# JuliaGenAI/ColBERT.jl

Hardware: AMD Instinct MI355X
Metric: queries/sec, top-1000 on 1M-passage corpus (higher is better)
Workload: dtype f32

## Files before the change

### colbert.jl_amd/csrc/approx_kernels.hpp

```cpp
#pragma once
#include <hip/hip_fp16.h>

#include <algorithm>

#include "common.hpp"
#include "search_kernels.hpp"

namespace clb {

typedef __bf16 bf16x8 __attribute__((ext_vector_type(8)));
typedef uint32_t u32x4 __attribute__((ext_vector_type(4)));
typedef uint32_t u32x4_a4 __attribute__((ext_vector_type(4), aligned(4)));
typedef float f32x4_a4 __attribute__((ext_vector_type(4), aligned(4)));

constexpr float kEpsSafety = 1.25f;

inline bool approx_supported(int dim, int nbits) { return dim == kDim && nbits == 2; }
inline size_t approx_cells_bytes(int64_t B, int64_t K, int64_t ) { return (size_t)B * K * 16 * 4 + 2048; }

__device__ __forceinline__ uint32_t f32_to_bf16_rne(float f) {
    const uint32_t u = __float_as_uint(f);
    return (u + 0x7fffu + ((u >> 16) & 1u)) >> 16;
}
__device__ __forceinline__ uint32_t pack_bf16(float lo, float hi) {
// ... 1213 lines not shown
    float rb_max;
    float dw_rn;
    float inv_qerr;
    float dc_max;
};

struct QueryBound { float eps_t, eps_sum; bool unsafe; };
__device__ __forceinline__ QueryBound query_bound(const float* __restrict__ Q, int b, int T, const ApproxConsts& ac,
                                                  float* s_qn, float* s_dq, const float4* __restrict__ tscale = nullptr,
                                                  float* s_aux = nullptr ,
                                                  bool cell8 = false) {
    const int tid = threadIdx.x;
    if (tid == 0) { *s_qn = 0.f; *s_dq = 0.f; }
    if (tscale && tid < 4) s_aux[tid] = 0.f;
    __syncthreads();
    {
        const int t = tid >> 5, part = tid & 31;
        float a = 0.f, dd = 0.f, d8 = 0.f;
        if (t < T) {
            const float4 v = *reinterpret_cast<const float4*>(Q + ((size_t)b * T + t) * kDim + 4 * part);
            a = fmaf(v.x, v.x, fmaf(v.y, v.y, fmaf(v.z, v.z, v.w * v.w)));
            const float dx = v.x - round_f16(v.x), dy = v.y - round_f16(v.y);
            const float dz = v.z - round_f16(v.z), dw = v.w - round_f16(v.w);
            dd = fmaf(dx, dx, fmaf(dy, dy, fmaf(dz, dz, dw * dw)));
            if (tscale && cell8) {
                const float4 ts = tscale[(size_t)b * 32 + t];
                const float sx = v.x * ts.y, sy = v.y * ts.y, sz = v.z * ts.y, sw = v.w * ts.y;
                const float ex = sx - round_f16(sx), ey = sy - round_f16(sy), ez = sz - round_f16(sz), ew = sw - round_f16(sw);
                d8 = fmaf(ex, ex, fmaf(ey, ey, fmaf(ez, ez, ew * ew)));
            }
        }
#pragma unroll
// ... 25 lines not shown
            const float dq8 = s_aux[0], step_max = s_aux[1];
            e_tab = e_f16 + 0.5005f * step_max + 8.f * u * amax;
            e_qr = 1.001f * ((dq8 + 2.f * u * qn) * ac.rb_max + qn * ac.dw_rn) +
                   2.f * 130.f * u * (amax + 255.f * step_max + qn * ac.rn_max) + 1280.f * u * step_max;
            bad8 = s_aux[2] != 0.f;
        }
    }
    const float eps_t = (ac.inv_max + ac.inv_qerr) * (e_tab + e_qr) + 1.01f * ac.inv_qerr * qn * (ac.cn_max + ac.rn_max) + 332.f * u * qn;
    QueryBound r;
    r.eps_t = eps_t;
    r.unsafe = !(qn * ac.cn_max < 3.0e4f) || !(qn < 6.0e4f)  || !(eps_t < 1.0e30f) || bad8;
    r.eps_sum = kEpsSafety * ((float)T * eps_t + 2.f * (float)T * (float)T * u * qn);
    return r;
}

static __global__ __launch_bounds__(1024) void select_margin_kernel(const float* __restrict__ scores,
                                                                   const int* __restrict__ ncand,
                                                                   const float* __restrict__ Q, int T, int k,
                                                                   size_t cand_cap, ApproxConsts ac,
                                                                   int* __restrict__ list, int* __restrict__ nlist,
                                                                   float* __restrict__ thresh,
                                                                   float* __restrict__ eps_pair,
                                                                   const float* __restrict__ tau_in = nullptr,
                                                                   int coarse_tau = 0,
                                                                   const float4* __restrict__ tscale = nullptr,
                                                                   int cell8 = 0) {
    __shared__ __attribute__((aligned(16))) int hist[256];
    __shared__ float s_aux[4];
    __shared__ int sh_scan[16];
    __shared__ int sh_big[2][8][16];
    __shared__ uint32_t s_prefix, s_kmin, s_kmax;
    __shared__ int s_remaining, s_run;
    __shared__ float s_qn, s_dq;
    const int b = blockIdx.x, tid = threadIdx.x;
    const int n = ncand[b];
    const float* sc = scores + (size_t)b * cand_cap;
    int* lst = list + (size_t)b * cand_cap;
    if (tid == 0) { s_prefix = 0u; s_remaining = n < k ? n : k; s_run = 0; }
    const int chunk = (n + 1023) >> 10;
    const int i0 = tid * chunk;
    const bool cached = chunk <= kSelCache;
    uint32_t ckey[kSelCache];
    if (cached) {
#pragma unroll
        for (int c = 0; c < kSelCache; ++c) ckey[c] = (c < chunk && i0 + c < n) ? f32_order_key(sc[i0 + c]) : 0u;
    }
    const QueryBound qb = query_bound(Q, b, T, ac, &s_qn, &s_dq, tscale, s_aux, cell8 != 0);
    float thr = kNegInf, tau_f = kNegInf, eps = 0.f;
    const bool unsafe = qb.unsafe;
    if (tid == 0) eps_pair[b] = unsafe ? __builtin_inff() : kEpsSafety * qb.eps_t;
#define CLB_SEL_FOR_EACH(...)                                                                   \
    if (cached) {                                                                               \
        _Pragma("unroll") for (int c = 0; c < kSelCache; ++c) {                                 \
            if (c >= chunk) break;                                                              \
            const int i = i0 + c;                                                               \
            const bool valid = i < n;                                                           \
            const uint32_t key = ckey[c];                                                       \
            __VA_ARGS__                                                                         \
        }                                                                                       \
    } else {    \
        _Pragma("unroll 4") for (int c = 0; c < chunk; ++c) {                                   \
            const int i = c * 1024 + tid;                                                       \
            const bool valid = i < n;                                                           \
            const uint32_t key = valid ? f32_order_key(sc[i]) : 0u;                             \
            __VA_ARGS__                                                                         \
// ... 148 lines not shown
                    st.shift = ns;
                }
            }
            __syncthreads();
        }
    }
    return st;
}

static __global__ __launch_bounds__(1024) void wide_minmax_kernel(const float* __restrict__ scores,
                                                                 const int* __restrict__ ncand,
                                                                 const float* __restrict__ Q, int T, size_t cand_cap,
                                                                 ApproxConsts ac, WideSel* __restrict__ wsel,
                                                                 float* __restrict__ eps_pair,
                                                                 const float4* __restrict__ tscale = nullptr,
                                                                 int cell8 = 0) {
    __shared__ uint32_t s_kmin, s_kmax;
    __shared__ float s_qn, s_dq, s_aux[4];
    const int b = blockIdx.y, g = blockIdx.x, tid = threadIdx.x;
    const int n = ncand[b];
    const float* sc = scores + (size_t)b * cand_cap;
    WideSel& w = wsel[b];
    if (tid == 0) { s_kmin = 0xffffffffu; s_kmax = 0u; }
    __syncthreads();
    if (g == 0) {
        const QueryBound qb = query_bound(Q, b, T, ac, &s_qn, &s_dq, tscale, s_aux, cell8 != 0);
        if (tid == 0) {
            eps_pair[b] = qb.unsafe ? __builtin_inff() : kEpsSafety * qb.eps_t;
            w.unsafe = qb.unsafe ? 1 : 0;
            w.eps_sum = qb.eps_sum;
        }
    }
    int lo, hi;
    wide_segment(n, g, lo, hi);
    uint32_t kmin = 0xffffffffu, kmax = 0u;
#pragma unroll 4
    for (int i = lo + tid; i < hi; i += 1024) {
        const uint32_t key = f32_order_key(sc[i]);
        kmin = key < kmin ? key : kmin;
        kmax = key > kmax ? key : kmax;
// ... 271 lines not shown
```

### colbert.jl_amd/csrc/search.hip

```cpp
#include <algorithm>
#include <atomic>
#include <cstdlib>
#include <cstring>
#include <numeric>

#include "approx_kernels.hpp"
#include "generic_kernels.hpp"
#include "search_kernels.hpp"
#include "sort.hpp"

using namespace clb;

namespace {

enum KernelId {
    KID_CENTROID_SCORES = 0,
    KID_TOPN,
    KID_MARK,
    KID_COMPACT,
    KID_SCORE_EXACT,
    KID_SCORE_APPROX,
    KID_SELECT,
    KID_ROWS,
    KID_TOPK,
// ... 34 lines not shown
    DevBuf bits;
};

struct Workspace {
    int64_t Bcap = 0, Tcap = 0, npcap = 0, kcap = 0;
    int64_t Ttuned = 0;
    size_t cand_cap = 0;
    int W = 0, nblk_bitmap = 0, topn_blocks = 0;
    bool x1_table = false;
    bool have_range = false;
    bool cell8 = false;
    size_t filt_cap = 0;
    size_t ivf_cap = 0;
    struct { bool valid = false; const float* dQ = nullptr; int64_t T = 0, B = 0, nprobe = 0, k = 0; void* stream = nullptr; } pending;
    DevBuf Qdev, cells, cells_q, partial, sel, bitmap, blocksum, ncand, cand, cand_hdr, scores, list, nlist, thresh,
        outp, outs, flags, stats, redo, rowmask, eps_pair, tokmax, tau_glob, wsel, bounds, tscale, rangep, cells8;
    DevBuf g_cells, g_keys, g_keys2, g_vals, g_vals2, g_scratch, g_sort_tmp;
};

constexpr int kWorkspaceSlots = 4;

struct clb_searcher {
    int device = 0;
    uint64_t serial = 0;
    int64_t dim = 0, K = 0, n_docs = 0, n_emb = 0, pid_offset = 0;
    int nbits = 0;
    int mode = 0;
    int wide_select = -1;
    bool approx_ok = false;
    bool bounds_synced = false;
    bool ivf_sorted = false;
// ... 68 lines not shown
            s->prof.chain_stream = st;
        } else {
            s->prof.failed = true;
            s->prof.chain = nullptr;
        }
    }
};

inline int token_tiles(int64_t T) { return T <= 32 ? 1 : T <= 64 ? 2 : 4; }
inline int64_t padded_nprobe(int64_t nprobe) { return nprobe <= 2 ? 2 : nprobe <= 8 ? 8 : nprobe <= 32 ? 32 : nprobe; }

inline bool cell8_rows(const clb_searcher* s) { return s->cell8 == 1 && s->approx_ok; }

void allow_large_topk_lds() {
    allow_dynamic_lds(reinterpret_cast<const void*>(topk_kernel), (int)(sizeof(unsigned long long) * kMaxTopK));
}

constexpr int64_t kSubBatch = 64;

int next_pow2(int x) {
    int p = 1;
    while (p < x) p <<= 1;
    return p;
}

int ensure_workspace_sized(clb_searcher* s, Workspace& w, int64_t B, int64_t T, int64_t nprobe, int64_t k, size_t filt_count) {
    const int64_t t_tuned = T <= 128 ? T : 0;
    if (B <= w.Bcap && T <= w.Tcap && t_tuned <= w.Ttuned && nprobe <= w.npcap && k <= w.kcap && filt_count <= w.filt_cap)
        return CLB_OK;
    CLB_HIP(hipDeviceSynchronize());
// ... 37 lines not shown
    CLB_TRY(w.scores.ensure(sizeof(float) * B * w.cand_cap));
    CLB_TRY(w.list.ensure(sizeof(int) * B * w.cand_cap));
    CLB_TRY(w.nlist.ensure(sizeof(int) * B));
    CLB_TRY(w.thresh.ensure(sizeof(float) * B * 2));
    CLB_TRY(w.outp.ensure(sizeof(int64_t) * B * k));
    CLB_TRY(w.outs.ensure(sizeof(float) * B * k));
    CLB_TRY(w.flags.ensure(sizeof(int) * B));
    if (!w.stats.p) {
        CLB_TRY(w.stats.ensure(sizeof(unsigned long long) * 8));
        CLB_HIP(hipMemset(w.stats.p, 0, sizeof(unsigned long long) * 8));
    }
    if (s->approx_ok && Ttuned > 0) {
        CLB_TRY(w.cells_q.ensure(approx_cells_bytes(B, s->K, Tpad)));
        CLB_TRY(w.rowmask.ensure(sizeof(unsigned long long) * 4 * B * w.cand_cap));
        CLB_TRY(w.eps_pair.ensure(sizeof(float) * B));
        CLB_TRY(w.tokmax.ensure(sizeof(uint16_t) * 32 * B * w.cand_cap));
    }
    w.Bcap = B; w.Tcap = T; w.Ttuned = Ttuned; w.npcap = nprobe; w.kcap = k;
    w.filt_cap = std::max(w.filt_cap, filt_count);
    CLB_HIP(hipStreamSynchronize(s->stream));
    return CLB_OK;
}

int ensure_workspace(clb_searcher* s, Workspace& w, int64_t B, int64_t T, int64_t nprobe, int64_t k, size_t filt_count = 0) {
    const int rc = ensure_workspace_sized(s, w, B, T, nprobe, k, filt_count);
    if (rc) {
        w.Bcap = 0;
        if (rc == CLB_ENOMEM && filt_count > w.filt_cap)
            return fail(CLB_EUNSUPPORTED, "no room for the candidate buffers of a filter of %zu passages (CLB_FILTER_ALL, %lld "
                                          "queries per pass): %s", filt_count, (long long)B, std::string(last_error()).c_str());
// ... 21 lines not shown
int select_by_sort(clb_searcher* s, Workspace& w, hipStream_t st, const float* cells, size_t stride_t, size_t stride_c,
                   int T, int nprobe, int NP, int* sel_b);

int select_top_nprobe(clb_searcher* s, Workspace& w, hipStream_t st, int B, int T, int Tpad, int nprobe) {
    const int NPs = (int)padded_nprobe(nprobe);
    if (NPs == 2) launch_topn<2>(s, w, st, B, Tpad);
    else if (NPs == 8) launch_topn<8>(s, w, st, B, Tpad);
    else if (NPs == 32) launch_topn<32>(s, w, st, B, Tpad);
    else
        for (int b = 0; b < B; ++b)
            CLB_TRY(select_by_sort(s, w, st, w.cells.as<float>() + (size_t)b * s->K * Tpad, 1, (size_t)Tpad, T, nprobe, NPs,
                                   w.sel.as<int>() + (size_t)b * Tpad * NPs));
    return CLB_OK;
}

int mark_and_compact(clb_searcher* s, Workspace& w, hipStream_t st, const Batch& q, int b0, int B, int Tpad, int NPs, bool timed);

int run_retrieve(clb_searcher* s, Workspace& w, hipStream_t st, const Batch& q) {
    const float* dQ = q.dQ;
    const int B = q.B, T = q.T, nprobe = q.nprobe;
    const int TT = token_tiles(T), Tpad = TT * 32;
    const int n_tiles = (int)((s->K + 31) / 32);
    const bool want_half = s->mode == 1 && s->approx_ok && T <= 32;
    w.x1_table = false;
    w.have_range = false;
    w.cell8 = false;
    if (nprobe <= 2 && T <= 32) {
        const bool mq = B >= 6;
        const int groups = (B + kMqQueries - 1) / kMqQueries;
        int gx = mq ? std::max(1, std::min(n_tiles, std::min(256, std::max(512 / groups, 16))))
                          : std::max(1, std::min(n_tiles / 2 + 1, std::min(256, std::max(1024 / std::max(1, B), 16))));
// ... 62 lines not shown
            Timed t(s, KID_CENTROID_SCORES, st);
            const int gx = std::max(1, std::min(n_tiles / 2 + 1, 2048 / std::max(1, B * TT)));
            hipLaunchKernelGGL(centroid_scores_kernel, dim3(gx, B * TT), dim3(128),
                               2 * 32 * kCentTileStride * sizeof(float), st, s->centroids.as<float>(), dQ,
                               w.cells.as<float>(), (int)s->K, T, TT, n_tiles);
        }
        {
            Timed t(s, KID_TOPN, st);
            CLB_TRY(select_top_nprobe(s, w, st, B, T, Tpad, nprobe));
        }
        s->prof.chain = nullptr;
        if (want_half)
            hipLaunchKernelGGL(cells_to_half_kernel, dim3(std::max(1, 1024 / B), B), dim3(256), 0, st,
                               w.cells.as<float>(), w.cells_q.as<uint32_t>(), (int)s->K);
    }
    return mark_and_compact(s, w, st, q, 0, B, Tpad, (int)padded_nprobe(nprobe), true);
}

FilterArgs filter_args(const Batch& q, int b0, int n) {
    FilterArgs fa{};
    for (int i = 0; i < n && i < kFilterQueries; ++i) fa.bits[i] = q.filt[b0 + i] ? q.filt[b0 + i]->bits.as<uint32_t>() : nullptr;
    fa.all = q.filt_all;
    return fa;
}

template <bool FILT>
int mark_and_compact_impl(clb_searcher* s, Workspace& w, hipStream_t st, const Batch& q, int b0, int B, int Tpad, int NPs,
                          bool timed) {
    static_assert(kScanBlock * kWordsPerThread == 1024, "mark_count_kernel writes 1024-word count blocks");
    static_assert(kSubBatch <= kFilterQueries, "the filter handles of a sub-batch travel in one kernel argument block");
    FilterOperand<FILT> fa{};
    if constexpr (FILT) fa = filter_args(q, b0, B);
    const int T = q.T, nprobe = q.nprobe;
    uint32_t* bitmap = w.bitmap.as<uint32_t>() + (size_t)b0 * w.W;
    int* blocksum = w.blocksum.as<int>() + (size_t)b0 * w.nblk_bitmap;
    uint32_t* cand = w.cand.as<uint32_t>() + (size_t)b0 * w.cand_cap;
    uint2* cand_hdr = w.cand_hdr.as<uint2>() + (size_t)b0 * w.cand_cap;
    int* ncand = w.ncand.as<int>() + b0;
    const int nslices = (w.nblk_bitmap + kMarkSliceBlocks - 1) / kMarkSliceBlocks;
    const int nslices_big = (w.nblk_bitmap + kMarkSliceBlocksBig - 1) / kMarkSliceBlocksBig;
    const bool sliced = (nslices <= 16 || s->ivf_sorted) && B >= 8;
    {
        Timed t(s, timed ? KID_MARK : -1, st);
// ... 5 lines not shown
            const int nb = T * nprobe * (nslices_big + 1);
            hipLaunchKernelGGL(slice_bounds_kernel, dim3((nb + 255) / 256, B), dim3(256), 0, st, w.sel.as<int>(),
                               s->ivf_off.as<uint32_t>(), s->ivf_pid.as<uint32_t>(), T, Tpad, NPs, nprobe, nslices_big,
                               (uint32_t)(kMarkSliceBlocksBig * 1024 * 32), w.bounds.as<uint32_t>());
            hipLaunchKernelGGL((mark_count_kernel<true, kMarkSliceBlocksBig, FILT>), dim3(nslices_big, B), dim3(1024), 0, st,
                               w.sel.as<int>(), s->ivf_off.as<uint32_t>(), s->ivf_pid.as<uint32_t>(), bitmap, blocksum, T, Tpad,
                               NPs, nprobe, w.W, w.nblk_bitmap, (const uint32_t*)w.bounds.as<uint32_t>(), fa);
        } else
            hipLaunchKernelGGL(mark_candidates_kernel<FILT>, dim3(T * nprobe, B), dim3(256), 0, st, w.sel.as<int>(),
                               s->ivf_off.as<uint32_t>(), s->ivf_pid.as<uint32_t>(), bitmap, T, Tpad, NPs, nprobe, w.W, fa);
    }
    {
        Timed t(s, timed ? KID_COMPACT : -1, st);
        if (!sliced)
            hipLaunchKernelGGL(bitmap_count_kernel<FILT>, dim3(w.nblk_bitmap, B), dim3(kScanBlock), 0, st, bitmap, blocksum, w.W, fa);
        if (FILT && (!sliced || q.filt_all))
            hipLaunchKernelGGL(bitmap_emit_kernel<FILT>, dim3(w.nblk_bitmap, B), dim3(kScanBlock), 0, st, bitmap, blocksum, cand,
                               s->doc_off.as<uint32_t>(), cand_hdr, w.W, w.cand_cap, ncand, fa);
        else
            hipLaunchKernelGGL(bitmap_emit_kernel<false>, dim3(w.nblk_bitmap, B), dim3(kScanBlock), 0, st, bitmap, blocksum, cand,
                               s->doc_off.as<uint32_t>(), cand_hdr, w.W, w.cand_cap, ncand);
    }
    CLB_HIP(hipGetLastError());
    return CLB_OK;
}

int mark_and_compact(clb_searcher* s, Workspace& w, hipStream_t st, const Batch& q, int b0, int B, int Tpad, int NPs, bool timed) {
    bool filt = false;
    for (int b = b0; q.filt && b < b0 + B; ++b) filt |= q.filt[b] != nullptr;
    return filt ? mark_and_compact_impl<true>(s, w, st, q, b0, B, Tpad, NPs, timed)
                : mark_and_compact_impl<false>(s, w, st, q, b0, B, Tpad, NPs, timed);
}

int check_search_args(clb_searcher* s, int64_t T, int64_t B, int64_t nprobe, int64_t k) {
    if (!s) return fail(CLB_EARGUMENT, "null searcher");
    if (T < 1) return fail(CLB_EARGUMENT, "query length must be >= 1");
    if (B < 1) return fail(CLB_EARGUMENT, "batch size must be >= 1");
    if (nprobe < 1 || nprobe > s->K) return fail(CLB_EBOUNDS, "nprobe=%lld outside 1..K=%lld (partialsortperm)", (long long)nprobe, (long long)s->K);
    if (k < 1) return fail(CLB_EBOUNDS, "k must be >= 1");
    if (T * nprobe > (int64_t)0x7fffffff / 4 || T * s->K > (int64_t)0x7fffffff) return fail(CLB_EUNSUPPORTED, "T * K too large");
    return CLB_OK;
}

int select_by_sort(clb_searcher* s, Workspace& w, hipStream_t st, const float* cells, size_t stride_t, size_t stride_c,
                   int T, int nprobe, int NP, int* sel_b) {
    const size_t n = (size_t)T * s->K;
// ... 18 lines not shown
    const int* lst = list ? list + (size_t)b * w.cand_cap : nullptr;
    const int* n_ptr = list ? nlist + b : w.ncand.as<int>() + b;
    CLB_TRY(w.g_keys.ensure(sizeof(uint64_t) * std::max(cap, 1)));
    CLB_TRY(w.g_keys2.ensure(sizeof(uint64_t) * std::max(cap, 1)));
    hipLaunchKernelGGL(generic_topk_keys_kernel, dim3((cap + 255) / 256), dim3(256), 0, st, sc, lst, n_ptr, cap,
                       w.g_keys.as<unsigned long long>());
    CLB_TRY(sort_keys_u64(w.g_keys.as<uint64_t>(), w.g_keys2.as<uint64_t>(), (size_t)cap, st, &w.g_sort_tmp));
    hipLaunchKernelGGL(generic_topk_emit_kernel, dim3((std::max(k, 1) + 255) / 256), dim3(256), 0, st,
                       w.g_keys2.as<unsigned long long>(), sc, w.cand.as<uint32_t>() + (size_t)b * w.cand_cap, lst, n_ptr,
                       w.ncand.as<int>() + b, k, s->pid_offset, q.d_out_pids + (size_t)b * k, q.d_out_scores + (size_t)b * k,
                       w.flags.as<int>() + b, q.d_n_cand ? q.d_n_cand + b : nullptr);
    CLB_HIP(hipGetLastError());
    return CLB_OK;
}

int launch_topk(clb_searcher* s, Workspace& w, hipStream_t st, const Batch& q, int b0, int n, const int* list, const int* nlist,
                int ranked) {
    if (q.k > kMaxTopK) {
        for (int b = b0; b < b0 + n; ++b) CLB_TRY(topk_by_sort(s, w, st, q, b, list, nlist));
        return CLB_OK;
    }
    const int kpow2 = next_pow2(q.k);
    allow_large_topk_lds();
    hipLaunchKernelGGL(topk_kernel, dim3(n), dim3(1024), sizeof(unsigned long long) * kpow2, st,
                       w.scores.as<float>() + (size_t)b0 * w.cand_cap, w.cand.as<uint32_t>() + (size_t)b0 * w.cand_cap,
                       w.ncand.as<int>() + b0, list ? list + (size_t)b0 * w.cand_cap : nullptr, list ? nlist + b0 : nullptr, q.k, kpow2,
                       w.cand_cap, s->pid_offset, q.d_out_pids + (size_t)b0 * q.k, q.d_out_scores + (size_t)b0 * q.k,
                       w.flags.as<int>() + b0, q.d_n_cand ? q.d_n_cand + b0 : nullptr, ranked);
    CLB_HIP(hipGetLastError());
    return CLB_OK;
}

int run_retrieve_general(clb_searcher* s, Workspace& w, hipStream_t st, const Batch& q, int b) {
    const int T = q.T, nprobe = q.nprobe;
    CLB_TRY(w.g_cells.ensure(sizeof(float) * (size_t)T * s->K));
    hipLaunchKernelGGL(generic_cells_kernel, dim3((unsigned)((s->K + 127) / 128), T), dim3(128), sizeof(float) * s->dim, st,
                       s->centroids.as<float>(), q.dQ + (size_t)b * T * s->dim, (int)s->dim, (int)s->K, w.g_cells.as<float>());
    CLB_TRY(select_by_sort(s, w, st, w.g_cells.as<float>(), (size_t)s->K, 1, T, nprobe, nprobe, w.sel.as<int>()));
    return mark_and_compact(s, w, st, q, b, 1, T, nprobe, false);
}

bool general_batched_ok(const clb_searcher* s, int T) { return s->dim % 4 == 0 && s->dim <= 256 && T <= 128; }

// ... 11 lines not shown
    const int B = q.B, T = q.T;
    s->prof.chain = nullptr;
    if (general_batched_ok(s, T)) {
        CLB_TRY(run_retrieve_general_batched(s, w, st, q));
        const dim3 grid((unsigned)std::max(64, 2048 / std::max(1, B)), (unsigned)B);
        const size_t lds = sizeof(float) * (((size_t)1 << s->nbits) + (size_t)T * (s->dim + 1));
        if (lds > 64 * 1024) {
            allow_dynamic_lds(reinterpret_cast<const void*>(generic_score_mfma_fast_kernel<32>), (int)lds);
            allow_dynamic_lds(reinterpret_cast<const void*>(generic_score_mfma_fast_kernel<64>), (int)lds);
        }
        auto score_kernel = s->dim <= 128 ? generic_score_mfma_fast_kernel<32> : generic_score_mfma_fast_kernel<64>;
        hipLaunchKernelGGL(score_kernel, grid, dim3(256), lds, st, s->centroids.as<float>(), s->weights.as<float>(),
                           s->codes0.as<uint32_t>(), s->residuals.as<uint8_t>(), w.cand_hdr.as<uint2>(), w.ncand.as<int>(), dQ,
                           (int)s->dim, s->nbits, T, w.cand_cap, w.scores.as<float>());
        CLB_HIP(hipGetLastError());
        return launch_topk(s, w, st, q, 0, B, nullptr, nullptr, 0);
    }
    const int grid = 1024;
    const size_t max_len = (size_t)std::max<int64_t>(s->max_doclen, 1);
    CLB_TRY(w.g_scratch.ensure(sizeof(float) * grid * max_len * s->dim));
    for (int b = 0; b < B; ++b) {
        CLB_TRY(run_retrieve_general(s, w, st, q, b));
        if (T <= 16 * kGenericMaxTokenGroups && s->dim % 4 == 0)
            hipLaunchKernelGGL(generic_score_mfma_kernel, dim3(grid), dim3(256), sizeof(float) * ((size_t)1 << s->nbits), st,
                               s->centroids.as<float>(), s->weights.as<float>(), s->codes0.as<uint32_t>(),
                               s->residuals.as<uint8_t>(), w.cand_hdr.as<uint2>() + (size_t)b * w.cand_cap,
                               w.ncand.as<int>() + b, dQ + (size_t)b * T * s->dim, (int)s->dim, s->nbits, T,
                               w.scores.as<float>() + (size_t)b * w.cand_cap);
        else
            hipLaunchKernelGGL(generic_score_kernel, dim3(grid), dim3(256), sizeof(float) * T, st, s->centroids.as<float>(),
                               s->weights.as<float>(), s->codes0.as<uint32_t>(), s->residuals.as<uint8_t>(),
                               w.cand_hdr.as<uint2>() + (size_t)b * w.cand_cap, w.ncand.as<int>() + b,
                               dQ + (size_t)b * T * s->dim, (int)s->dim, s->nbits, T, w.g_scratch.as<float>(), max_len,
                               w.scores.as<float>() + (size_t)b * w.cand_cap);
        CLB_HIP(hipGetLastError());
        CLB_TRY(launch_topk(s, w, st, q, b, 1, nullptr, nullptr, 0));
    }
    return CLB_OK;
}

constexpr size_t kWideSelectCap = 131072;

void launch_pass1(clb_searcher* s, Workspace& w, hipStream_t st, const float* dQ, dim3 grid, int B, int T) {
    auto kern = w.cell8 ? (s->gather_lds ? score_approx32_kernel<false, 1, true> : score_approx32_kernel<false, 0, true>)
                        : (s->gather_lds ? score_approx32_kernel<false, 1, false> : score_approx32_kernel<false, 0, false>);
    hipLaunchKernelGGL(kern, grid, dim3(kApproxThreads), 0, st, s->weights.as<float>(),
                       s->codeinv.as<uint32_t>(), s->residuals.as<uint8_t>(), s->cbits, s->inv_lo, s->inv_step, dQ,
                       w.cell8 ? w.cells8.as<uint32_t>() : w.cells_q.as<uint32_t>(), w.cand_hdr.as<uint2>(), w.ncand.as<int>(),
                       w.scores.as<float>(), (int)s->K, T, B, w.cand_cap, w.tokmax.as<uint16_t>(), (const int*)nullptr,
                       (const int*)nullptr, (const float*)nullptr, (unsigned long long*)nullptr,
                       (const float4*)w.tscale.as<float4>());
}
inline float bound_dc(const clb_searcher* s, const Workspace& w) {
    return (w.x1_table || (s->bounds_synced && s->s1_x1 != 0 && s->cent_f16.p)) ? s->dc_f16 : 0.f;
}
int launch_select(clb_searcher* s, Workspace& w, hipStream_t st, const Batch& q, const float* tau_in, bool coarse_tau = false) {
    const float* dQ = q.dQ;
    const int B = q.B, T = q.T, k = q.k;
    const size_t most = q.filt && q.filt_all ? std::max(w.ivf_cap, q.filt_now) : w.ivf_cap;
    const bool wide = s->wide_select == 1 || (s->wide_select < 0 && most >= kWideSelectCap);
    if (!wide) {
        ApproxConsts ac = s->approx_consts;
        ac.dc_max = bound_dc(s, w);
        hipLaunchKernelGGL(select_margin_kernel, dim3(B), dim3(1024), 0, st, w.scores.as<float>(), w.ncand.as<int>(), dQ, T, k,
                           w.cand_cap, ac, w.list.as<int>(), w.nlist.as<int>(), w.thresh.as<float>(),
                           w.eps_pair.as<float>(), tau_in, coarse_tau ? 1 : 0,
                           w.have_range ? (const float4*)w.tscale.as<float4>() : (const float4*)nullptr, w.cell8 ? 1 : 0);
        return CLB_OK;
    }
    CLB_TRY(w.wsel.ensure(sizeof(WideSel) * B));
    CLB_HIP(hipMemsetAsync(w.wsel.p, 0, sizeof(WideSel) * B, st));
    const dim3 grid(kWideBlocks, B);
    ApproxConsts acw = s->approx_consts;
    acw.dc_max = bound_dc(s, w);
    hipLaunchKernelGGL(wide_minmax_kernel, grid, dim3(1024), 0, st, w.scores.as<float>(), w.ncand.as<int>(), dQ, T, w.cand_cap,
                       acw, w.wsel.as<WideSel>(), w.eps_pair.as<float>(),
                       w.have_range ? (const float4*)w.tscale.as<float4>() : (const float4*)nullptr, w.cell8 ? 1 : 0);
    if (!tau_in)
        for (int pass = 0; pass < 4; ++pass)
            hipLaunchKernelGGL(wide_hist_kernel, grid, dim3(1024), 0, st, w.scores.as<float>(), w.ncand.as<int>(), k, w.cand_cap,
                               w.wsel.as<WideSel>(), pass);
    hipLaunchKernelGGL(wide_count_kernel, grid, dim3(1024), 0, st, w.scores.as<float>(), w.ncand.as<int>(), k, w.cand_cap,
                       w.wsel.as<WideSel>(), tau_in);
    hipLaunchKernelGGL(wide_emit_kernel, grid, dim3(1024), 0, st, w.scores.as<float>(), w.ncand.as<int>(), k, w.cand_cap,
                       (const WideSel*)w.wsel.as<WideSel>(), tau_in, w.list.as<int>(), w.nlist.as<int>(), w.thresh.as<float>());
    return CLB_OK;
}

int run_search(clb_searcher* s, Workspace& w, hipStream_t st, const Batch& q) {
    const float* dQ = q.dQ;
    const int B = q.B, T = q.T, k = q.k, phase = q.phase;
    const bool two_pass = s->mode == 1 && s->approx_ok && T <= 32;
// ... 53 lines not shown
        if (subset)
            hipLaunchKernelGGL(score_exact_flat_kernel, dim3(std::max(1, kFlatGx / B), B), dim3(256), 0, st, s->centroids.as<float>(),
                               s->weights.as<float>(), s->codes0.as<uint32_t>(), s->residuals.as<uint8_t>(),
                               w.cand_hdr.as<uint2>(), dQ, w.scores.as<float>(), T, w.cand_cap, list, nlist,
                               w.rowmask.as<unsigned long long>());
        else
            switch (s->nbits) {
                case 1: launch_score_exact<1>(s, w, st, dQ, B, T, list, nlist, gx); break;
                case 2: launch_score_exact<2>(s, w, st, dQ, B, T, list, nlist, gx); break;
                case 4: launch_score_exact<4>(s, w, st, dQ, B, T, list, nlist, gx); break;
                default: return fail(CLB_EUNSUPPORTED, "nbits=%d not supported by the HIP search path", s->nbits);
            }
    }
    if (k <= kMaxTopK) {
        Timed t(s, KID_TOPK, st);
        const int ranked = list != nullptr;
        if (ranked)
            hipLaunchKernelGGL(topk_rank_kernel, dim3(kRankBlocks, B), dim3(1024), 0, st, w.scores.as<float>(),
                               w.cand.as<uint32_t>(), w.ncand.as<int>(), list, nlist, k, w.cand_cap, s->pid_offset,
                               q.d_out_pids, q.d_out_scores, w.flags.as<int>(), q.d_n_cand);
        CLB_TRY(launch_topk(s, w, st, q, 0, B, list, nlist, ranked));
    } else {
        s->prof.chain = nullptr;
        CLB_TRY(launch_topk(s, w, st, q, 0, B, list, nlist, 0));
    }
    if (s->prof.counters) {
        hipLaunchKernelGGL(batch_stats_kernel, dim3(32, B), dim3(256), 0, st, w.cand.as<uint32_t>(),
                           w.ncand.as<int>(), list, nlist, s->doc_off.as<uint32_t>(), w.cand_cap,
                           w.stats.as<unsigned long long>(),
                           subset ? w.rowmask.as<unsigned long long>() : (const unsigned long long*)nullptr);
    }
    CLB_HIP(hipGetLastError());
    return CLB_OK;
}

int check_filters(const clb_searcher* s, const clb_filter* const* filters, int64_t B, int scope, size_t* filt_count) {
    *filt_count = 0;
    if (scope != CLB_FILTER_CANDIDATES && scope != CLB_FILTER_ALL)
        return fail(CLB_EARGUMENT, "scope must be CLB_FILTER_CANDIDATES (0) or CLB_FILTER_ALL (1), got %d", scope);
// ... 730 lines not shown
```

### colbert.jl_amd/csrc/search_kernels.hpp

```cpp
#pragma once
#include <hip/hip_fp16.h>

#include <type_traits>

#include "common.hpp"

namespace clb {

typedef float f32x16 __attribute__((ext_vector_type(16)));
typedef float f32x4 __attribute__((ext_vector_type(4)));

constexpr int kDim = 128;
constexpr int kCentTileStride = 132;
constexpr int kMaxTopK = 16384;

static __global__ __launch_bounds__(128) void centroid_scores_kernel(const float* __restrict__ C,
                                                               const float* __restrict__ Q,
                                                               float* __restrict__ cells, int K, int T,
                                                               int TT, int n_tiles) {
    extern __shared__ __attribute__((aligned(16))) float lds[];
    const int wave = threadIdx.x >> 6, lane = threadIdx.x & 63;
    const int i = lane & 31, h = lane >> 5;
    const int b = blockIdx.y / TT, tt = blockIdx.y % TT;
    const int Tpad = TT * 32;
// ... 301 lines not shown
        const uint32_t* fw = fa.bits[b];
        const bool from_filter = fw && fa.all;
#pragma unroll
        for (int j = 0; j < kWordsPerThread; ++j)
            if (w0 + j < W) cnt += __popc(!fw ? bm[w0 + j] : from_filter ? fw[w0 + j] : bm[w0 + j] & fw[w0 + j]);
    } else {
#pragma unroll
    for (int j = 0; j < kWordsPerThread; ++j)
        if (w0 + j < W) cnt += __popc(bm[w0 + j]);
    }
    int total;
    (void)block_exclusive_scan_256(cnt, sh, total);
    if (threadIdx.x == 0) blocksum[(size_t)b * gridDim.x + blockIdx.x] = total;
}

template <bool FILT = false>
static __global__ __launch_bounds__(kScanBlock) void bitmap_emit_kernel(uint32_t* __restrict__ bitmap,
                                                                 const int* __restrict__ blockcnt,
                                                                 uint32_t* __restrict__ cand,
                                                                 const uint32_t* __restrict__ doc_off,
                                                                 uint2* __restrict__ cand_hdr, int W,
                                                                 size_t cand_cap, int* __restrict__ ncand,
                                                                 FilterOperand<FILT> fa = {}) {
    __shared__ int sh[8];
    const int b = blockIdx.y;
    int before = 0;
    {
        const int* bc = blockcnt + (size_t)b * gridDim.x;
        const int upto = blockIdx.x == 0 ? (int)gridDim.x : (int)blockIdx.x;
        int part = 0;
        for (int i = threadIdx.x; i < upto; i += kScanBlock) part += bc[i];
        int total_;
        (void)block_exclusive_scan_256(part, sh, total_);
        if (blockIdx.x == 0) { if (threadIdx.x == 0) ncand[b] = total_; }
        else before = total_;
    }
    uint32_t* bm = bitmap + (size_t)b * W;
    const int w0 = (blockIdx.x * kScanBlock + threadIdx.x) * kWordsPerThread;
// ... 27 lines not shown
        bool clear = x != 0u;
        if constexpr (FILT) clear = marked[j] != 0u;
        if (clear) bm[w0 + j] = 0u;
        while (x) {
            const int bit = __ffs((int)x) - 1;
            x &= x - 1;
            if ((size_t)pos < cand_cap) {
                const uint32_t pid = (uint32_t)((w0 + j) * 32 + bit);
                out[pos] = pid;
                const uint32_t o = doc_off[pid];
                hdr[pos] = make_uint2(o, doc_off[pid + 1] - o);
            }
            ++pos;
        }
    }
}

static __global__ __launch_bounds__(256) void filter_mark_kernel(const int64_t* __restrict__ pids, int64_t n, int64_t pid_offset,
                                                                 int n_docs, uint32_t* __restrict__ bits, int* __restrict__ err) {
    const int64_t i = (int64_t)blockIdx.x * 256 + threadIdx.x;
    if (i >= n) return;
    const int64_t p = pids[i] - pid_offset - 1;
    if (p < 0 || p >= (int64_t)n_docs) { atomicOr(err, 1); return; }
    atomicOr(&bits[p >> 5], 1u << (p & 31));
}
static __global__ __launch_bounds__(256) void filter_count_kernel(uint32_t* __restrict__ bits, int W, int n_docs,
                                                                  unsigned long long* __restrict__ count) {
    int c = 0;
    for (int w = blockIdx.x * 256 + threadIdx.x; w < W; w += gridDim.x * 256) {
        uint32_t x = bits[w];
// ... 567 lines not shown
                                                     valid && (key & himask_) == prefix_);)                 \
                __syncthreads();                                                                            \
                if (tid < 64) radix_pick(hist, s_remaining, prefix_, shift_, &s_prefix, &s_remaining);      \
                __syncthreads();                                                                            \
                if (shift_ == 0 || ++passes_ >= (LIMIT)) break;                                             \
                const int ns_ = shift_ > 8 ? shift_ - 8 : 0;                                                \
                width_ = shift_ - ns_;                                                                      \
                shift_ = ns_;                                                                               \
            }                                                                                               \
        }                                                                                                   \
    }

constexpr int kRankMax = 4096;
constexpr int kRankBlocks = 8;

static __global__ __launch_bounds__(1024) void topk_kernel(const float* __restrict__ scores,
                                                    const uint32_t* __restrict__ cand,
                                                    const int* __restrict__ ncand,
                                                    const int* __restrict__ list,
                                                    const int* __restrict__ nlist, int k, int kpow2,
                                                    size_t cand_cap, int64_t pid_offset,
                                                    int64_t* __restrict__ out_pids,
                                                    float* __restrict__ out_scores,
                                                    int* __restrict__ short_flag,
                                                    int64_t* __restrict__ n_cand_out ,
                                                    int ranked_elsewhere = 0) {
    extern __shared__ __attribute__((aligned(16))) unsigned long long skeys[];
    __shared__ __attribute__((aligned(16))) int hist[256];
    __shared__ int sh_scan[32];
    __shared__ uint32_t s_prefix, s_kmin, s_kmax;
    __shared__ int s_remaining;
    const int b = blockIdx.x, tid = threadIdx.x;
    const int n = list ? nlist[b] : ncand[b];
    if (ranked_elsewhere && list && n <= kRankMax) return;
    const float* sc = scores + (size_t)b * cand_cap;
    const int* lst = list ? list + (size_t)b * cand_cap : nullptr;
    const int keff = n < k ? n : k;
    int kp = 1;
    while (kp < keff) kp <<= 1;
    kp = kp < kpow2 ? kp : kpow2;
    if (tid == 0) {
        short_flag[b] = n < k ? 1 : 0;
        if (n_cand_out) n_cand_out[b] = ncand[b];
    }

    const int chunk = (n + 1023) >> 10;
    const int i0 = tid * chunk;
    const bool cached = chunk <= kSelCache;
    uint32_t ckey[kSelCache];
    int cslot[kSelCache];
    if (cached) {
#pragma unroll
        for (int c = 0; c < kSelCache; ++c) {
            const int i = i0 + c;
            const bool valid = c < chunk && i < n;
            cslot[c] = valid ? (lst ? lst[i] : i) : 0;
            ckey[c] = valid ? f32_order_key(sc[cslot[c]]) : 0u;
        }
    }
#define CLB_SEL_FOR_EACH(...)                                                                   \
    if (cached) {                                                                               \
        _Pragma("unroll") for (int c = 0; c < kSelCache; ++c) {                                 \
            if (c >= chunk) break;                                                              \
            const bool valid = i0 + c < n;                                                      \
            const int slot = cslot[c];                                                          \
            const uint32_t key = ckey[c];                                                       \
            (void)slot;                                                                         \
            __VA_ARGS__                                                                         \
        }                                                                                       \
    } else {                                                                                    \
        for (int c = 0; c < chunk; ++c) {                                                       \
            const bool valid = i0 + c < n;                                                      \
            const int slot = valid ? (lst ? lst[i0 + c] : i0 + c) : 0;                          \
            const uint32_t key = valid ? f32_order_key(sc[slot]) : 0u;                          \
            (void)slot;                                                                         \
            __VA_ARGS__                                                                         \
        }                                                                                       \
// ... 67 lines not shown
    const uint32_t* cnd = cand + (size_t)b * cand_cap;
    for (int i = tid; i < k; i += 1024) {
        int64_t pid = 0;
        float s = kNegInf;
        if (i < keff) {
            const unsigned long long key = skeys[i];
            const uint32_t slot = 0xffffffffu - (uint32_t)(key & 0xffffffffull);
            pid = pid_offset + (int64_t)cnd[slot] + 1;
            s = sc[slot];
        }
        out_pids[(size_t)b * k + i] = pid;
        out_scores[(size_t)b * k + i] = s;
    }
}

static __global__ __launch_bounds__(1024) void topk_rank_kernel(const float* __restrict__ scores,
                                                                const uint32_t* __restrict__ cand,
                                                                const int* __restrict__ ncand,
                                                                const int* __restrict__ list,
                                                                const int* __restrict__ nlist, int k, size_t cand_cap,
                                                                int64_t pid_offset, int64_t* __restrict__ out_pids,
                                                                float* __restrict__ out_scores,
                                                                int* __restrict__ short_flag,
                                                                int64_t* __restrict__ n_cand_out ) {
    __shared__ __attribute__((aligned(16))) unsigned long long keys[kRankMax];
    __shared__ int ranks[256];
    const int b = blockIdx.y, g = blockIdx.x, tid = threadIdx.x;
    const int n = nlist[b];
    if (n > kRankMax) return;
    const float* sc = scores + (size_t)b * cand_cap;
    const int* lst = list + (size_t)b * cand_cap;
    const int keff = n < k ? n : k;
    if (g == 0) {
        if (tid == 0) {
            short_flag[b] = n < k ? 1 : 0;
            if (n_cand_out) n_cand_out[b] = ncand[b];
        }
        for (int i = keff + tid; i < k; i += 1024) {
            out_pids[(size_t)b * k + i] = 0;
            out_scores[(size_t)b * k + i] = kNegInf;
        }
    }
    for (int i = tid; i < n; i += 1024) {
        const int slot = lst[i];
// ... 167 lines not shown
```

Baseline: 30920.

## Fuse query-bound computation into bitmap emit and merge topk fallback into rank kernel

Computes the per-query error bound once in the last block of the bitmap emit kernel and stores eps_pair and eps_sum, so the select-margin and wide-minmax kernels read the stored value instead of recomputing it. The ranked top-k path now handles lists larger than kRankMax inside topk_rank_kernel using a shared select-sort helper. That removes the second topk_kernel launch, which previously ran after the rank kernel and exited early for small lists. The cost is extra work in the emit kernel's tail block and dynamic LDS for the rank kernel.

Result: no change. 30870 (-0.2%).

```diff
diff --git a/colbert.jl_amd/csrc/approx_kernels.hpp b/colbert.jl_amd/csrc/approx_kernels.hpp
--- a/colbert.jl_amd/csrc/approx_kernels.hpp
+++ b/colbert.jl_amd/csrc/approx_kernels.hpp
@@ -1251,8 +1251,8 @@
     if (tid == 0) { *s_qn = 0.f; *s_dq = 0.f; }
     if (tscale && tid < 4) s_aux[tid] = 0.f;
     __syncthreads();
-    {
-        const int t = tid >> 5, part = tid & 31;
+    for (int t = tid >> 5; t < 32; t += (int)(blockDim.x >> 5)) {
+        const int part = tid & 31;
         float a = 0.f, dd = 0.f, d8 = 0.f;
         if (t < T) {
             const float4 v = *reinterpret_cast<const float4*>(Q + ((size_t)b * T + t) * kDim + 4 * part);
@@ -1308,6 +1308,23 @@
     return r;
 }
 
+struct QueryBoundJob {
+    const float* Q;
+    const float4* tscale;
+    float* eps_pair;
+    float* eps_sum;
+    ApproxConsts ac;
+    int T, cell8;
+    __device__ __forceinline__ void operator()(int b) const {
+        __shared__ float s_qn, s_dq, s_aux[4];
+        const QueryBound qb = query_bound(Q, b, T, ac, &s_qn, &s_dq, tscale, s_aux, cell8 != 0);
+        if (threadIdx.x == 0) {
+            eps_pair[b] = qb.unsafe ? __builtin_inff() : kEpsSafety * qb.eps_t;
+            eps_sum[b] = qb.unsafe ? __builtin_inff() : qb.eps_sum;
+        }
+    }
+};
+
 static __global__ __launch_bounds__(1024) void select_margin_kernel(const float* __restrict__ scores,
                                                                    const int* __restrict__ ncand,
                                                                    const float* __restrict__ Q, int T, int k,
@@ -1318,7 +1335,8 @@
                                                                    const float* __restrict__ tau_in = nullptr,
                                                                    int coarse_tau = 0,
                                                                    const float4* __restrict__ tscale = nullptr,
-                                                                   int cell8 = 0) {
+                                                                   int cell8 = 0,
+                                                                   const float* __restrict__ eps_sum_in = nullptr) {
     __shared__ __attribute__((aligned(16))) int hist[256];
     __shared__ float s_aux[4];
     __shared__ int sh_scan[16];
@@ -1339,10 +1357,16 @@
 #pragma unroll
         for (int c = 0; c < kSelCache; ++c) ckey[c] = (c < chunk && i0 + c < n) ? f32_order_key(sc[i0 + c]) : 0u;
     }
-    const QueryBound qb = query_bound(Q, b, T, ac, &s_qn, &s_dq, tscale, s_aux, cell8 != 0);
+    QueryBound qb;
+    if (eps_sum_in) {
+        qb.eps_sum = eps_sum_in[b];
+        qb.unsafe = qb.eps_sum == __builtin_inff();
+    } else {
+        qb = query_bound(Q, b, T, ac, &s_qn, &s_dq, tscale, s_aux, cell8 != 0);
+        if (tid == 0) eps_pair[b] = qb.unsafe ? __builtin_inff() : kEpsSafety * qb.eps_t;
+    }
     float thr = kNegInf, tau_f = kNegInf, eps = 0.f;
     const bool unsafe = qb.unsafe;
-    if (tid == 0) eps_pair[b] = unsafe ? __builtin_inff() : kEpsSafety * qb.eps_t;
 #define CLB_SEL_FOR_EACH(...)                                                                   \
     if (cached) {                                                                               \
         _Pragma("unroll") for (int c = 0; c < kSelCache; ++c) {                                 \
@@ -1521,7 +1545,8 @@
                                                                  ApproxConsts ac, WideSel* __restrict__ wsel,
                                                                  float* __restrict__ eps_pair,
                                                                  const float4* __restrict__ tscale = nullptr,
-                                                                 int cell8 = 0) {
+                                                                 int cell8 = 0,
+                                                                 const float* __restrict__ eps_sum_in = nullptr) {
     __shared__ uint32_t s_kmin, s_kmax;
     __shared__ float s_qn, s_dq, s_aux[4];
     const int b = blockIdx.y, g = blockIdx.x, tid = threadIdx.x;
@@ -1530,7 +1555,13 @@
     WideSel& w = wsel[b];
     if (tid == 0) { s_kmin = 0xffffffffu; s_kmax = 0u; }
     __syncthreads();
-    if (g == 0) {
+    if (g == 0 && eps_sum_in) {
+        if (tid == 0) {
+            const float e = eps_sum_in[b];
+            w.unsafe = e == __builtin_inff() ? 1 : 0;
+            w.eps_sum = e;
+        }
+    } else if (g == 0) {
         const QueryBound qb = query_bound(Q, b, T, ac, &s_qn, &s_dq, tscale, s_aux, cell8 != 0);
         if (tid == 0) {
             eps_pair[b] = qb.unsafe ? __builtin_inff() : kEpsSafety * qb.eps_t;
diff --git a/colbert.jl_amd/csrc/search.hip b/colbert.jl_amd/csrc/search.hip
--- a/colbert.jl_amd/csrc/search.hip
+++ b/colbert.jl_amd/csrc/search.hip
@@ -72,7 +72,7 @@
     size_t ivf_cap = 0;
     struct { bool valid = false; const float* dQ = nullptr; int64_t T = 0, B = 0, nprobe = 0, k = 0; void* stream = nullptr; } pending;
     DevBuf Qdev, cells, cells_q, partial, sel, bitmap, blocksum, ncand, cand, cand_hdr, scores, list, nlist, thresh,
-        outp, outs, flags, stats, redo, rowmask, eps_pair, tokmax, tau_glob, wsel, bounds, tscale, rangep, cells8;
+        outp, outs, flags, stats, redo, rowmask, eps_pair, eps_sum, tokmax, tau_glob, wsel, bounds, tscale, rangep, cells8;
     DevBuf g_cells, g_keys, g_keys2, g_vals, g_vals2, g_scratch, g_sort_tmp;
 };
 
@@ -171,6 +171,7 @@
 
 void allow_large_topk_lds() {
     allow_dynamic_lds(reinterpret_cast<const void*>(topk_kernel), (int)(sizeof(unsigned long long) * kMaxTopK));
+    allow_dynamic_lds(reinterpret_cast<const void*>(topk_rank_kernel), (int)(sizeof(unsigned long long) * kMaxTopK));
 }
 
 constexpr int64_t kSubBatch = 64;
@@ -238,6 +239,7 @@
         CLB_TRY(w.cells_q.ensure(approx_cells_bytes(B, s->K, Tpad)));
         CLB_TRY(w.rowmask.ensure(sizeof(unsigned long long) * 4 * B * w.cand_cap));
         CLB_TRY(w.eps_pair.ensure(sizeof(float) * B));
+        CLB_TRY(w.eps_sum.ensure(sizeof(float) * B));
         CLB_TRY(w.tokmax.ensure(sizeof(uint16_t) * 32 * B * w.cand_cap));
     }
     w.Bcap = B; w.Tcap = T; w.Ttuned = Ttuned; w.npcap = nprobe; w.kcap = k;
@@ -289,7 +291,9 @@
     return CLB_OK;
 }
 
-int mark_and_compact(clb_searcher* s, Workspace& w, hipStream_t st, const Batch& q, int b0, int B, int Tpad, int NPs, bool timed);
+int mark_and_compact(clb_searcher* s, Workspace& w, hipStream_t st, const Batch& q, int b0, int B, int Tpad, int NPs, bool timed,
+                     const QueryBoundJob* bound = nullptr);
+inline float bound_dc(const clb_searcher* s, const Workspace& w);
 
 int run_retrieve(clb_searcher* s, Workspace& w, hipStream_t st, const Batch& q) {
     const float* dQ = q.dQ;
@@ -382,7 +386,11 @@
             hipLaunchKernelGGL(cells_to_half_kernel, dim3(std::max(1, 1024 / B), B), dim3(256), 0, st,
                                w.cells.as<float>(), w.cells_q.as<uint32_t>(), (int)s->K);
     }
-    return mark_and_compact(s, w, st, q, 0, B, Tpad, (int)padded_nprobe(nprobe), true);
+    if (!want_half) return mark_and_compact(s, w, st, q, 0, B, Tpad, (int)padded_nprobe(nprobe), true);
+    QueryBoundJob bound{dQ, w.have_range ? (const float4*)w.tscale.as<float4>() : (const float4*)nullptr, w.eps_pair.as<float>(),
+                        w.eps_sum.as<float>(), s->approx_consts, T, w.cell8 ? 1 : 0};
+    bound.ac.dc_max = bound_dc(s, w);
+    return mark_and_compact(s, w, st, q, 0, B, Tpad, (int)padded_nprobe(nprobe), true, &bound);
 }
 
 FilterArgs filter_args(const Batch& q, int b0, int n) {
@@ -394,7 +402,7 @@
 
 template <bool FILT>
 int mark_and_compact_impl(clb_searcher* s, Workspace& w, hipStream_t st, const Batch& q, int b0, int B, int Tpad, int NPs,
-                          bool timed) {
+                          bool timed, const QueryBoundJob* bound) {
     static_assert(kScanBlock * kWordsPerThread == 1024, "mark_count_kernel writes 1024-word count blocks");
     static_assert(kSubBatch <= kFilterQueries, "the filter handles of a sub-batch travel in one kernel argument block");
     FilterOperand<FILT> fa{};
@@ -430,22 +438,32 @@
         Timed t(s, timed ? KID_COMPACT : -1, st);
         if (!sliced)
             hipLaunchKernelGGL(bitmap_count_kernel<FILT>, dim3(w.nblk_bitmap, B), dim3(kScanBlock), 0, st, bitmap, blocksum, w.W, fa);
-        if (FILT && (!sliced || q.filt_all))
-            hipLaunchKernelGGL(bitmap_emit_kernel<FILT>, dim3(w.nblk_bitmap, B), dim3(kScanBlock), 0, st, bitmap, blocksum, cand,
-                               s->doc_off.as<uint32_t>(), cand_hdr, w.W, w.cand_cap, ncand, fa);
+        const dim3 grid(w.nblk_bitmap, B);
+        const uint32_t* doc_off = s->doc_off.as<uint32_t>();
+        if (FILT && (!sliced || q.filt_all)) {
+            if (bound)
+                hipLaunchKernelGGL((bitmap_emit_kernel<FILT, QueryBoundJob>), grid, dim3(kScanBlock), 0, st, bitmap, blocksum, cand,
+                                   doc_off, cand_hdr, w.W, w.cand_cap, ncand, fa, *bound);
+            else
+                hipLaunchKernelGGL(bitmap_emit_kernel<FILT>, grid, dim3(kScanBlock), 0, st, bitmap, blocksum, cand, doc_off,
+                                   cand_hdr, w.W, w.cand_cap, ncand, fa);
+        } else if (bound)
+            hipLaunchKernelGGL((bitmap_emit_kernel<false, QueryBoundJob>), grid, dim3(kScanBlock), 0, st, bitmap, blocksum, cand,
+                               doc_off, cand_hdr, w.W, w.cand_cap, ncand, FilterOperand<false>{}, *bound);
         else
-            hipLaunchKernelGGL(bitmap_emit_kernel<false>, dim3(w.nblk_bitmap, B), dim3(kScanBlock), 0, st, bitmap, blocksum, cand,
-                               s->doc_off.as<uint32_t>(), cand_hdr, w.W, w.cand_cap, ncand);
+            hipLaunchKernelGGL(bitmap_emit_kernel<false>, grid, dim3(kScanBlock), 0, st, bitmap, blocksum, cand, doc_off,
+                               cand_hdr, w.W, w.cand_cap, ncand);
     }
     CLB_HIP(hipGetLastError());
     return CLB_OK;
 }
 
-int mark_and_compact(clb_searcher* s, Workspace& w, hipStream_t st, const Batch& q, int b0, int B, int Tpad, int NPs, bool timed) {
+int mark_and_compact(clb_searcher* s, Workspace& w, hipStream_t st, const Batch& q, int b0, int B, int Tpad, int NPs, bool timed,
+                     const QueryBoundJob* bound) {
     bool filt = false;
     for (int b = b0; q.filt && b < b0 + B; ++b) filt |= q.filt[b] != nullptr;
-    return filt ? mark_and_compact_impl<true>(s, w, st, q, b0, B, Tpad, NPs, timed)
-                : mark_and_compact_impl<false>(s, w, st, q, b0, B, Tpad, NPs, timed);
+    return filt ? mark_and_compact_impl<true>(s, w, st, q, b0, B, Tpad, NPs, timed, bound)
+                : mark_and_compact_impl<false>(s, w, st, q, b0, B, Tpad, NPs, timed, bound);
 }
 
 int check_search_args(clb_searcher* s, int64_t T, int64_t B, int64_t nprobe, int64_t k) {
@@ -494,8 +512,7 @@
     return CLB_OK;
 }
 
-int launch_topk(clb_searcher* s, Workspace& w, hipStream_t st, const Batch& q, int b0, int n, const int* list, const int* nlist,
-                int ranked) {
+int launch_topk(clb_searcher* s, Workspace& w, hipStream_t st, const Batch& q, int b0, int n, const int* list, const int* nlist) {
     if (q.k > kMaxTopK) {
         for (int b = b0; b < b0 + n; ++b) CLB_TRY(topk_by_sort(s, w, st, q, b, list, nlist));
         return CLB_OK;
@@ -506,7 +523,7 @@
                        w.scores.as<float>() + (size_t)b0 * w.cand_cap, w.cand.as<uint32_t>() + (size_t)b0 * w.cand_cap,
                        w.ncand.as<int>() + b0, list ? list + (size_t)b0 * w.cand_cap : nullptr, list ? nlist + b0 : nullptr, q.k, kpow2,
                        w.cand_cap, s->pid_offset, q.d_out_pids + (size_t)b0 * q.k, q.d_out_scores + (size_t)b0 * q.k,
-                       w.flags.as<int>() + b0, q.d_n_cand ? q.d_n_cand + b0 : nullptr, ranked);
+                       w.flags.as<int>() + b0, q.d_n_cand ? q.d_n_cand + b0 : nullptr);
     CLB_HIP(hipGetLastError());
     return CLB_OK;
 }
@@ -548,7 +565,7 @@
                            s->codes0.as<uint32_t>(), s->residuals.as<uint8_t>(), w.cand_hdr.as<uint2>(), w.ncand.as<int>(), dQ,
                            (int)s->dim, s->nbits, T, w.cand_cap, w.scores.as<float>());
         CLB_HIP(hipGetLastError());
-        return launch_topk(s, w, st, q, 0, B, nullptr, nullptr, 0);
+        return launch_topk(s, w, st, q, 0, B, nullptr, nullptr);
     }
     const int grid = 1024;
     const size_t max_len = (size_t)std::max<int64_t>(s->max_doclen, 1);
@@ -568,7 +585,7 @@
                                dQ + (size_t)b * T * s->dim, (int)s->dim, s->nbits, T, w.g_scratch.as<float>(), max_len,
                                w.scores.as<float>() + (size_t)b * w.cand_cap);
         CLB_HIP(hipGetLastError());
-        CLB_TRY(launch_topk(s, w, st, q, b, 1, nullptr, nullptr, 0));
+        CLB_TRY(launch_topk(s, w, st, q, b, 1, nullptr, nullptr));
     }
     return CLB_OK;
 }
@@ -599,7 +616,8 @@
         hipLaunchKernelGGL(select_margin_kernel, dim3(B), dim3(1024), 0, st, w.scores.as<float>(), w.ncand.as<int>(), dQ, T, k,
                            w.cand_cap, ac, w.list.as<int>(), w.nlist.as<int>(), w.thresh.as<float>(),
                            w.eps_pair.as<float>(), tau_in, coarse_tau ? 1 : 0,
-                           w.have_range ? (const float4*)w.tscale.as<float4>() : (const float4*)nullptr, w.cell8 ? 1 : 0);
+                           w.have_range ? (const float4*)w.tscale.as<float4>() : (const float4*)nullptr, w.cell8 ? 1 : 0,
+                           (const float*)w.eps_sum.as<float>());
         return CLB_OK;
     }
     CLB_TRY(w.wsel.ensure(sizeof(WideSel) * B));
@@ -609,7 +627,8 @@
     acw.dc_max = bound_dc(s, w);
     hipLaunchKernelGGL(wide_minmax_kernel, grid, dim3(1024), 0, st, w.scores.as<float>(), w.ncand.as<int>(), dQ, T, w.cand_cap,
                        acw, w.wsel.as<WideSel>(), w.eps_pair.as<float>(),
-                       w.have_range ? (const float4*)w.tscale.as<float4>() : (const float4*)nullptr, w.cell8 ? 1 : 0);
+                       w.have_range ? (const float4*)w.tscale.as<float4>() : (const float4*)nullptr, w.cell8 ? 1 : 0,
+                       (const float*)w.eps_sum.as<float>());
     if (!tau_in)
         for (int pass = 0; pass < 4; ++pass)
             hipLaunchKernelGGL(wide_hist_kernel, grid, dim3(1024), 0, st, w.scores.as<float>(), w.ncand.as<int>(), k, w.cand_cap,
@@ -693,15 +712,19 @@
     }
     if (k <= kMaxTopK) {
         Timed t(s, KID_TOPK, st);
-        const int ranked = list != nullptr;
-        if (ranked)
-            hipLaunchKernelGGL(topk_rank_kernel, dim3(kRankBlocks, B), dim3(1024), 0, st, w.scores.as<float>(),
-                               w.cand.as<uint32_t>(), w.ncand.as<int>(), list, nlist, k, w.cand_cap, s->pid_offset,
+        if (list) {
+            const int kpow2 = next_pow2(k);
+            allow_large_topk_lds();
+            hipLaunchKernelGGL(topk_rank_kernel, dim3(kRankBlocks, B), dim3(1024),
+                               sizeof(unsigned long long) * std::max(kRankMax, kpow2), st, w.scores.as<float>(),
+                               w.cand.as<uint32_t>(), w.ncand.as<int>(), list, nlist, k, kpow2, w.cand_cap, s->pid_offset,
                                q.d_out_pids, q.d_out_scores, w.flags.as<int>(), q.d_n_cand);
-        CLB_TRY(launch_topk(s, w, st, q, 0, B, list, nlist, ranked));
+        } else {
+            CLB_TRY(launch_topk(s, w, st, q, 0, B, list, nlist));
+        }
     } else {
         s->prof.chain = nullptr;
-        CLB_TRY(launch_topk(s, w, st, q, 0, B, list, nlist, 0));
+        CLB_TRY(launch_topk(s, w, st, q, 0, B, list, nlist));
     }
     if (s->prof.counters) {
         hipLaunchKernelGGL(batch_stats_kernel, dim3(32, B), dim3(256), 0, st, w.cand.as<uint32_t>(),
diff --git a/colbert.jl_amd/csrc/search_kernels.hpp b/colbert.jl_amd/csrc/search_kernels.hpp
--- a/colbert.jl_amd/csrc/search_kernels.hpp
+++ b/colbert.jl_amd/csrc/search_kernels.hpp
@@ -339,14 +339,17 @@
     if (threadIdx.x == 0) blocksum[(size_t)b * gridDim.x + blockIdx.x] = total;
 }
 
-template <bool FILT = false>
+struct NoJob {
+    __device__ __forceinline__ void operator()(int) const {}
+};
+template <bool FILT = false, class JOB = NoJob>
 static __global__ __launch_bounds__(kScanBlock) void bitmap_emit_kernel(uint32_t* __restrict__ bitmap,
                                                                  const int* __restrict__ blockcnt,
                                                                  uint32_t* __restrict__ cand,
                                                                  const uint32_t* __restrict__ doc_off,
                                                                  uint2* __restrict__ cand_hdr, int W,
                                                                  size_t cand_cap, int* __restrict__ ncand,
-                                                                 FilterOperand<FILT> fa = {}) {
+                                                                 FilterOperand<FILT> fa = {}, JOB job = {}) {
     __shared__ int sh[8];
     const int b = blockIdx.y;
     int before = 0;
@@ -404,6 +407,7 @@
             ++pos;
         }
     }
+    if (blockIdx.x == gridDim.x - 1) job(b);
 }
 
 static __global__ __launch_bounds__(256) void filter_mark_kernel(const int64_t* __restrict__ pids, int64_t n, int64_t pid_offset,
@@ -1001,25 +1005,18 @@
 constexpr int kRankMax = 4096;
 constexpr int kRankBlocks = 8;
 
-static __global__ __launch_bounds__(1024) void topk_kernel(const float* __restrict__ scores,
-                                                    const uint32_t* __restrict__ cand,
-                                                    const int* __restrict__ ncand,
-                                                    const int* __restrict__ list,
-                                                    const int* __restrict__ nlist, int k, int kpow2,
-                                                    size_t cand_cap, int64_t pid_offset,
-                                                    int64_t* __restrict__ out_pids,
-                                                    float* __restrict__ out_scores,
-                                                    int* __restrict__ short_flag,
-                                                    int64_t* __restrict__ n_cand_out ,
-                                                    int ranked_elsewhere = 0) {
-    extern __shared__ __attribute__((aligned(16))) unsigned long long skeys[];
+template <int CACHE>
+__device__ __forceinline__ void topk_select_sort(const int b, const int n, unsigned long long* skeys,
+                                                 const float* __restrict__ scores, const uint32_t* __restrict__ cand,
+                                                 const int* __restrict__ ncand, const int* __restrict__ list, int k,
+                                                 int kpow2, size_t cand_cap, int64_t pid_offset,
+                                                 int64_t* __restrict__ out_pids, float* __restrict__ out_scores,
+                                                 int* __restrict__ short_flag, int64_t* __restrict__ n_cand_out) {
     __shared__ __attribute__((aligned(16))) int hist[256];
     __shared__ int sh_scan[32];
     __shared__ uint32_t s_prefix, s_kmin, s_kmax;
     __shared__ int s_remaining;
-    const int b = blockIdx.x, tid = threadIdx.x;
-    const int n = list ? nlist[b] : ncand[b];
-    if (ranked_elsewhere && list && n <= kRankMax) return;
+    const int tid = threadIdx.x;
     const float* sc = scores + (size_t)b * cand_cap;
     const int* lst = list ? list + (size_t)b * cand_cap : nullptr;
     const int keff = n < k ? n : k;
@@ -1033,12 +1030,12 @@
 
     const int chunk = (n + 1023) >> 10;
     const int i0 = tid * chunk;
-    const bool cached = chunk <= kSelCache;
-    uint32_t ckey[kSelCache];
-    int cslot[kSelCache];
+    const bool cached = chunk <= CACHE;
+    uint32_t ckey[CACHE];
+    int cslot[CACHE];
     if (cached) {
 #pragma unroll
-        for (int c = 0; c < kSelCache; ++c) {
+        for (int c = 0; c < CACHE; ++c) {
             const int i = i0 + c;
             const bool valid = c < chunk && i < n;
             cslot[c] = valid ? (lst ? lst[i] : i) : 0;
@@ -1047,7 +1044,7 @@
     }
 #define CLB_SEL_FOR_EACH(...)                                                                   \
     if (cached) {                                                                               \
-        _Pragma("unroll") for (int c = 0; c < kSelCache; ++c) {                                 \
+        _Pragma("unroll") for (int c = 0; c < CACHE; ++c) {                                 \
             if (c >= chunk) break;                                                              \
             const bool valid = i0 + c < n;                                                      \
             const int slot = cslot[c];                                                          \
@@ -1145,20 +1142,42 @@
     }
 }
 
+static __global__ __launch_bounds__(1024) void topk_kernel(const float* __restrict__ scores,
+                                                    const uint32_t* __restrict__ cand,
+                                                    const int* __restrict__ ncand,
+                                                    const int* __restrict__ list,
+                                                    const int* __restrict__ nlist, int k, int kpow2,
+                                                    size_t cand_cap, int64_t pid_offset,
+                                                    int64_t* __restrict__ out_pids,
+                                                    float* __restrict__ out_scores,
+                                                    int* __restrict__ short_flag,
+                                                    int64_t* __restrict__ n_cand_out ) {
+    extern __shared__ __attribute__((aligned(16))) unsigned long long skeys[];
+    const int b = blockIdx.x;
+    topk_select_sort<kSelCache>(b, list ? nlist[b] : ncand[b], skeys, scores, cand, ncand, list, k, kpow2, cand_cap, pid_offset,
+                     out_pids, out_scores, short_flag, n_cand_out);
+}
+
 static __global__ __launch_bounds__(1024) void topk_rank_kernel(const float* __restrict__ scores,
                                                                 const uint32_t* __restrict__ cand,
                                                                 const int* __restrict__ ncand,
                                                                 const int* __restrict__ list,
-                                                                const int* __restrict__ nlist, int k, size_t cand_cap,
-                                                                int64_t pid_offset, int64_t* __restrict__ out_pids,
+                                                                const int* __restrict__ nlist, int k, int kpow2,
+                                                                size_t cand_cap, int64_t pid_offset,
+                                                                int64_t* __restrict__ out_pids,
                                                                 float* __restrict__ out_scores,
                                                                 int* __restrict__ short_flag,
                                                                 int64_t* __restrict__ n_cand_out ) {
-    __shared__ __attribute__((aligned(16))) unsigned long long keys[kRankMax];
+    extern __shared__ __attribute__((aligned(16))) unsigned long long keys[];
     __shared__ int ranks[256];
     const int b = blockIdx.y, g = blockIdx.x, tid = threadIdx.x;
     const int n = nlist[b];
-    if (n > kRankMax) return;
+    if (n > kRankMax) {
+        if (g == 0)
+            topk_select_sort<8>(b, n, keys, scores, cand, ncand, list, k, kpow2, cand_cap, pid_offset, out_pids, out_scores,
+                             short_flag, n_cand_out);
+        return;
+    }
     const float* sc = scores + (size_t)b * cand_cap;
     const int* lst = list + (size_t)b * cand_cap;
     const int keff = n < k ? n : k;
```
